# brade31919/radar_depth

Hardware: AMD Instinct MI355X
Metric: training samples/sec, resnet18_latefusion b=16 450x800 rgbd, 1/2/4/8 MI355X (higher is better)
Workload: dtype f32

## Files before the change

radar_depth_amd/csrc/norm_act.hip:

```cpp
#include "conv_internal.h"

namespace rd {

__global__ __launch_bounds__(256) void bn_finalize_kernel(const float* __restrict__ part, int n_tiles, int ld, int c0, double count,
                                                          const float* __restrict__ gamma, const float* __restrict__ beta,
                                                          float eps, float momentum, float* running_mean, float* running_var,
                                                          int64_t* nbt, float* mean, float* invstd, float* scale, float* shift) {
    const int c = blockIdx.x;
    double s = 0.0, q = 0.0;
    int t = threadIdx.x;
    for (; t + 3 * 256 < n_tiles; t += 4 * 256) {
        float a[4], b[4];
#pragma unroll
        for (int k = 0; k < 4; ++k) {
            a[k] = part[((size_t)(t + k * 256) * 2 + 0) * ld + c0 + c];
            b[k] = part[((size_t)(t + k * 256) * 2 + 1) * ld + c0 + c];
        }
#pragma unroll
        for (int k = 0; k < 4; ++k) { s += (double)a[k]; q += (double)b[k]; }
    }
    for (; t < n_tiles; t += 256) {
        s += (double)part[((size_t)t * 2 + 0) * ld + c0 + c];
        q += (double)part[((size_t)t * 2 + 1) * ld + c0 + c];
    }
// ... 49 lines not shown
}

static inline int rows_per_block(int64_t M) {
    int64_t r = cdiv64(M, 2048);
    return (int)(r < 64 ? 64 : r);
}
static inline int bwd_rows_per_block(int64_t M, int C) {
    const int RL = 256 / (C / 4) > 0 ? 256 / (C / 4) : 1;
    int64_t r = cdiv64(M, 2048);
    const int64_t lo = 4 * RL < 64 ? 4 * RL : 64;
    return (int)(r < lo ? lo : r);
}

template <int NS>
__device__ __forceinline__ void block_reduce_store(float4 (&acc)[NS], int Q, int RL, int q, int rl, bool active, float* out,
                                                   int C, float* sm) {
    if (active) {
#pragma unroll
        for (int s = 0; s < NS; ++s) *reinterpret_cast<float4*>(sm + ((size_t)(rl * NS + s) * Q + q) * 4) = acc[s];
    }
    rd_sync();
    for (int e = threadIdx.x; e < NS * Q * 4; e += blockDim.x) {
        const int s = e / (Q * 4), c = e - s * (Q * 4);
        float v = 0.f;
        for (int r = 0; r < RL; ++r) v += sm[(size_t)(r * NS + s) * Q * 4 + c];
        out[(size_t)s * C + c] = v;
    }
}

template <typename T>
__global__ __launch_bounds__(256) void bn_stats_kernel(const T* __restrict__ x, int64_t M, int C, int ldx, int RPB,
                                                       float* __restrict__ part) {
    extern __shared__ float sm[];
    const int Q = C >> 2, RL = 256 / Q;
    const int q = threadIdx.x % Q, rl = threadIdx.x / Q;
    const bool active = rl < RL;
    const int64_t r0 = (int64_t)blockIdx.x * RPB, r1 = r0 + RPB < M ? r0 + RPB : M;
    float4 acc[2] = {make_float4(0, 0, 0, 0), make_float4(0, 0, 0, 0)};
    if (active)
        for (int64_t r = r0 + rl; r < r1; r += RL) {
            const float4 v = ld4(x + r * ldx + q * 4);
            acc[0].x += v.x; acc[0].y += v.y; acc[0].z += v.z; acc[0].w += v.w;
            acc[1].x += v.x * v.x; acc[1].y += v.y * v.y; acc[1].z += v.z * v.z; acc[1].w += v.w * v.w;
        }
    block_reduce_store<2>(acc, Q, RL, q, rl, active, part + (size_t)blockIdx.x * 2 * C, C, sm);
}

template <typename T>
__global__ __launch_bounds__(256) void bn_act_kernel(const T* __restrict__ x1, int ldx1, const float* __restrict__ s1,
                                                     const float* __restrict__ t1, const T* __restrict__ x2, int ldx2,
                                                     const float* __restrict__ s2, const float* __restrict__ t2,
                                                     T* __restrict__ y, int ldy, int64_t M, int C, int act,
                                                     unsigned short* __restrict__ pc, int64_t pplane) {
    const int Q = C >> 2;
    const int lq = quad_log2(Q);
    const int64_t total = M * Q;
    for (int64_t e = (int64_t)blockIdx.x * blockDim.x + threadIdx.x; e < total; e += (int64_t)gridDim.x * blockDim.x) {
        int64_t r;
        int c;
        split_quad(e, Q, lq, r, c);
        const float4 v = ld4(x1 + r * ldx1 + c);
        const float4 a = *reinterpret_cast<const float4*>(s1 + c);
        const float4 b = *reinterpret_cast<const float4*>(t1 + c);
        float4 z = make_float4(fmaf(a.x, v.x, b.x), fmaf(a.y, v.y, b.y), fmaf(a.z, v.z, b.z), fmaf(a.w, v.w, b.w));
        if (x2) {
            float4 u = ld4(x2 + r * ldx2 + c);
            if (s2) {
                const float4 a2 = *reinterpret_cast<const float4*>(s2 + c);
                const float4 b2 = *reinterpret_cast<const float4*>(t2 + c);
                u = make_float4(fmaf(a2.x, u.x, b2.x), fmaf(a2.y, u.y, b2.y), fmaf(a2.z, u.z, b2.z), fmaf(a2.w, u.w, b2.w));
            }
            z.x += u.x; z.y += u.y; z.z += u.z; z.w += u.w;
        }
        z.x = act_fwd(z.x, act); z.y = act_fwd(z.y, act); z.z = act_fwd(z.z, act); z.w = act_fwd(z.w, act);
        st4(y + r * ldy + c, z);
        if (pc) store_pieces4(pc, pplane, M, r, c, z);
    }
}

template <typename T>
__global__ __launch_bounds__(256) void bn_bwd_reduce_kernel(const T* __restrict__ dy, int lddy, const T* __restrict__ y,
                                                            int ldy, const T* __restrict__ x1, int ldx1,
                                                            const float* __restrict__ m1, const T* __restrict__ x2, int ldx2,
                                                            const float* __restrict__ m2, T* __restrict__ g, int ldg,
                                                            int64_t M, int C, int act, int RPB, float* __restrict__ part,
                                                            const float* __restrict__ s1, const float* __restrict__ t1,
                                                            const float* __restrict__ s2, const float* __restrict__ t2) {
    extern __shared__ float sm[];
    const int Q = C >> 2, RL = 256 / Q;
    const int q = threadIdx.x % Q, rl = threadIdx.x / Q;
    const bool active = rl < RL;
    const int64_t r0 = (int64_t)blockIdx.x * RPB, r1 = r0 + RPB < M ? r0 + RPB : M;
    float4 acc[3] = {make_float4(0, 0, 0, 0), make_float4(0, 0, 0, 0), make_float4(0, 0, 0, 0)};
    if (active) {
        const int c = q * 4;
        const float4 mu1 = x1 ? *reinterpret_cast<const float4*>(m1 + c) : make_float4(0, 0, 0, 0);
        const float4 mu2 = x2 ? *reinterpret_cast<const float4*>(m2 + c) : make_float4(0, 0, 0, 0);
        const bool from_x = act != RD_ACT_NONE && !y;
        const float4 sa = from_x ? *reinterpret_cast<const float4*>(s1 + c) : make_float4(0, 0, 0, 0);
        const float4 sb = from_x ? *reinterpret_cast<const float4*>(t1 + c) : make_float4(0, 0, 0, 0);
        const bool from_x2 = from_x && x2 && s2;
        const float4 sa2 = from_x2 ? *reinterpret_cast<const float4*>(s2 + c) : make_float4(0, 0, 0, 0);
        const float4 sb2 = from_x2 ? *reinterpret_cast<const float4*>(t2 + c) : make_float4(0, 0, 0, 0);
        for (int64_t r = r0 + rl; r < r1; r += RL) {
            float4 gv = ld4(dy + r * lddy + c);
            float4 v = make_float4(0, 0, 0, 0), v2 = make_float4(0, 0, 0, 0);
            if (x1) v = ld4(x1 + r * ldx1 + c);
            if (x2) v2 = ld4(x2 + r * ldx2 + c);
            if (act != RD_ACT_NONE) {
                float4 yv;
                if (from_x) {
                    yv = make_float4(fmaf(sa.x, v.x, sb.x), fmaf(sa.y, v.y, sb.y), fmaf(sa.z, v.z, sb.z), fmaf(sa.w, v.w, sb.w));
                    if (from_x2) {
                        yv.x += fmaf(sa2.x, v2.x, sb2.x); yv.y += fmaf(sa2.y, v2.y, sb2.y);
                        yv.z += fmaf(sa2.z, v2.z, sb2.z); yv.w += fmaf(sa2.w, v2.w, sb2.w);
                    }
                } else yv = ld4(y + r * ldy + c);
                gv.x *= act_grad_from_out(yv.x, act); gv.y *= act_grad_from_out(yv.y, act);
                gv.z *= act_grad_from_out(yv.z, act); gv.w *= act_grad_from_out(yv.w, act);
            }
            if (g) st4(g + r * ldg + c, gv);
            acc[0].x += gv.x; acc[0].y += gv.y; acc[0].z += gv.z; acc[0].w += gv.w;
            if (x1) {
                acc[1].x += gv.x * (v.x - mu1.x); acc[1].y += gv.y * (v.y - mu1.y);
                acc[1].z += gv.z * (v.z - mu1.z); acc[1].w += gv.w * (v.w - mu1.w);
            }
            if (x2) {
                acc[2].x += gv.x * (v2.x - mu2.x); acc[2].y += gv.y * (v2.y - mu2.y);
                acc[2].z += gv.z * (v2.z - mu2.z); acc[2].w += gv.w * (v2.w - mu2.w);
            }
        }
    }
    block_reduce_store<3>(acc, Q, RL, q, rl, active, part + (size_t)blockIdx.x * 3 * C, C, sm);
}

__global__ __launch_bounds__(256) void bn_bwd_coeffs_kernel(const float* __restrict__ part, int n_tiles, int C, int which,
                                                            double count, const float* __restrict__ gamma,
                                                            const float* __restrict__ invstd, float* dgamma, float* dbeta,
                                                            float* coef) {
    const int c = blockIdx.x;
    double s0 = 0.0, s1 = 0.0;
    int t = threadIdx.x;
    for (; t + 3 * 256 < n_tiles; t += 4 * 256) {
        float a[4], b[4];
#pragma unroll
        for (int k = 0; k < 4; ++k) {
            a[k] = part[((size_t)(t + k * 256) * 3 + 0) * C + c];
            b[k] = part[((size_t)(t + k * 256) * 3 + which) * C + c];
        }
#pragma unroll
        for (int k = 0; k < 4; ++k) { s0 += (double)a[k]; s1 += (double)b[k]; }
    }
    for (; t < n_tiles; t += 256) {
        s0 += (double)part[((size_t)t * 3 + 0) * C + c];
        s1 += (double)part[((size_t)t * 3 + which) * C + c];
    }
    __shared__ double sh[2][4];
    s0 = wave_sum_d(s0);
    s1 = wave_sum_d(s1);
    const int w = threadIdx.x >> 6;
    if ((threadIdx.x & 63) == 0) { sh[0][w] = s0; sh[1][w] = s1; }
    rd_sync();
    if (threadIdx.x == 0) {
// ... 231 lines not shown
                    st4(g + ix, d4);
                } else if (g) {
                    st4(g + ix, o4);
                }
                if (part) {
                    acc[0].x += o4.x; acc[0].y += o4.y; acc[0].z += o4.z; acc[0].w += o4.w;
                    acc[1].x += o4.x * (vv.x - mu.x); acc[1].y += o4.y * (vv.y - mu.y);
                    acc[1].z += o4.z * (vv.z - mu.z); acc[1].w += o4.w * (vv.w - mu.w);
                }
            }
    }
    if (part) block_reduce_store<3>(acc, Q, 256 / Q, threadIdx.x % Q, threadIdx.x / Q, true, part + (size_t)blockIdx.x * 3 * C, C, sm);
}

static int ew_grid(int64_t elems) {
    int64_t g = cdiv64(elems, 256);
    const int64_t cap = (int64_t)num_cus() * 16;
    if (g > cap) g = cap;
    return (int)(g < 1 ? 1 : g);
}

static inline bool quads_ok(int C) { return C >= 4 && C % 4 == 0; }
static inline bool ld_ok(const void* p, int ld, int C) { return !p || (ld % 4 == 0 && ld >= C); }

}
using namespace rd;

extern "C" int rd_bn_finalize(const float* stat_partial, int32_t n_tiles, int32_t ld, int32_t c0, int32_t C, int64_t count, const float* gamma,
                              const float* beta, float eps, float momentum, float* running_mean, float* running_var,
                              int64_t* nbt, float* mean, float* invstd, float* scale, float* shift, void* stream) {
    RD_CHECK_ARG(n_tiles > 0 && quads_ok(C) && count > 0, "bn_finalize: bad shape (n_tiles %d, C %d)", n_tiles, C);
    RD_CHECK_ARG(c0 >= 0 && ld % 4 == 0 && (int64_t)c0 + C <= ld, "bn_finalize: channels [%d, %d + %d) outside ld = %d", c0, c0, C, ld);
    RD_CHECK_ARG(stat_partial && gamma && beta && mean && invstd && scale && shift && (!running_mean == !running_var),
                 "bn_finalize: null pointer");
    hipLaunchKernelGGL(bn_finalize_kernel, dim3(C), dim3(256), 0, static_cast<hipStream_t>(stream), stat_partial, n_tiles, ld, c0,
                       (double)count, gamma, beta, eps, momentum, running_mean, running_var, nbt, mean, invstd, scale, shift);
    RD_CHECK_LAUNCH("bn_finalize_kernel");
    return RD_OK;
}

extern "C" int rd_bn_eval_coeffs(int32_t C, const float* gamma, const float* beta, const float* running_mean,
                                 const float* running_var, float eps, float* scale, float* shift, void* stream) {
    RD_CHECK_ARG(C > 0 && gamma && beta && running_mean && running_var && scale && shift, "bn_eval_coeffs: bad arguments");
    hipLaunchKernelGGL(bn_eval_coeffs_kernel, dim3(cdiv(C, 256)), dim3(256), 0, static_cast<hipStream_t>(stream), C, gamma, beta,
                       running_mean, running_var, eps, scale, shift);
    RD_CHECK_LAUNCH("bn_eval_coeffs_kernel");
// ... 54 lines not shown
}
extern "C" int rd_bn_act_t(int32_t dtype, const void* x1, int32_t ldx1, const float* scale1, const float* shift1, const void* x2, int32_t ldx2, const float* scale2, const float* shift2, void* y, int32_t ldy, int64_t M, int32_t C, int32_t act, void* stream) {
    if (dtype == RD_DTYPE_F32) return rd_bn_act_T<float>(static_cast<const float*>(x1), ldx1, scale1, shift1, static_cast<const float*>(x2), ldx2, scale2, shift2, static_cast<float*>(y), ldy, M, C, act, stream);
    if (dtype == RD_DTYPE_BF16) return rd_bn_act_T<bf16s>(static_cast<const bf16s*>(x1), ldx1, scale1, shift1, static_cast<const bf16s*>(x2), ldx2, scale2, shift2, static_cast<bf16s*>(y), ldy, M, C, act, stream);
    rd::set_error("rd_bn_act_t: bad dtype %d", dtype);
    return RD_EINVAL;
}

template <typename T>
static int bn_bwd_reduce_impl(const T* dy, int32_t lddy, const T* y, int32_t ldy, const T* x1, int32_t ldx1,
                              const float* mean1, const T* x2, int32_t ldx2, const float* mean2, T* g, int32_t ldg,
                              int64_t M, int32_t C, int32_t act, float* red_partial, const float* scale1, const float* shift1,
                              void* stream, const float* scale2 = nullptr, const float* shift2 = nullptr, bool two_bn = false) {
    RD_CHECK_ARG(M > 0 && quads_ok(C) && C <= 1024, "bn_bwd_reduce: bad shape (C %d)", C);
    RD_CHECK_ARG(lddy % 4 == 0 && lddy >= C && ld_ok(y, ldy, C) && ld_ok(x1, ldx1, C) && ld_ok(x2, ldx2, C) && ld_ok(g, ldg, C),
                 "bn_bwd_reduce: bad stride");
    RD_CHECK_ARG(dy && red_partial, "bn_bwd_reduce: null pointer");
    RD_CHECK_ARG(!two_bn || (x1 && x2 && scale1 && shift1 && scale2 && shift2 && act != RD_ACT_NONE), "bn_bwd_reduce_x2: bad arguments");
    RD_CHECK_ARG(act == RD_ACT_NONE || y || (scale1 && shift1 && x1 && (!x2 || (scale2 && shift2))),
                 "bn_bwd_reduce: activation needs y (or the scale/shift of every operand)");
    RD_CHECK_ARG((!x1 || mean1) && (!x2 || mean2), "bn_bwd_reduce: x without mean");
    const int RPB = bwd_rows_per_block(M, C), grid = (int)cdiv64(M, RPB);
    const int Q = C / 4, RL = 256 / Q;
    hipLaunchKernelGGL(bn_bwd_reduce_kernel, dim3(grid), dim3(256), (size_t)RL * 3 * C * sizeof(float),
                       static_cast<hipStream_t>(stream), dy, lddy, y, ldy, x1, ldx1, mean1, x2, ldx2, mean2, g, ldg, M, C, act, RPB,
                       red_partial, scale1, shift1, scale2, shift2);
    RD_CHECK_LAUNCH("bn_bwd_reduce_kernel");
    return RD_OK;
}
template <typename T>
static int rd_bn_bwd_reduce_T(const T* dy, int32_t lddy, const T* y, int32_t ldy, const T* x1, int32_t ldx1, const float* mean1, const T* x2, int32_t ldx2, const float* mean2, T* g, int32_t ldg, int64_t M, int32_t C, int32_t act, float* red_partial, void* stream) {
    return bn_bwd_reduce_impl<T>(dy, lddy, y, ldy, x1, ldx1, mean1, x2, ldx2, mean2, g, ldg, M, C, act, red_partial, nullptr, nullptr, stream);
}
extern "C" int rd_bn_bwd_reduce(const float* dy, int32_t lddy, const float* y, int32_t ldy, const float* x1, int32_t ldx1, const float* mean1, const float* x2, int32_t ldx2, const float* mean2, float* g, int32_t ldg, int64_t M, int32_t C, int32_t act, float* red_partial, void* stream) {
    return rd_bn_bwd_reduce_T<float>(dy, lddy, y, ldy, x1, ldx1, mean1, x2, ldx2, mean2, g, ldg, M, C, act, red_partial, stream);
}
extern "C" int rd_bn_bwd_reduce_t(int32_t dtype, const void* dy, int32_t lddy, const void* y, int32_t ldy, const void* x1, int32_t ldx1, const float* mean1, const void* x2, int32_t ldx2, const float* mean2, void* g, int32_t ldg, int64_t M, int32_t C, int32_t act, float* red_partial, void* stream) {
    if (dtype == RD_DTYPE_F32) return rd_bn_bwd_reduce_T<float>(static_cast<const float*>(dy), lddy, static_cast<const float*>(y), ldy, static_cast<const float*>(x1), ldx1, mean1, static_cast<const float*>(x2), ldx2, mean2, static_cast<float*>(g), ldg, M, C, act, red_partial, stream);
    if (dtype == RD_DTYPE_BF16) return rd_bn_bwd_reduce_T<bf16s>(static_cast<const bf16s*>(dy), lddy, static_cast<const bf16s*>(y), ldy, static_cast<const bf16s*>(x1), ldx1, mean1, static_cast<const bf16s*>(x2), ldx2, mean2, static_cast<bf16s*>(g), ldg, M, C, act, red_partial, stream);
    rd::set_error("rd_bn_bwd_reduce_t: bad dtype %d", dtype);
    return RD_EINVAL;
}
template <typename T>
static int rd_bn_bwd_reduce_x_T(const T* dy, int32_t lddy, const T* x1, int32_t ldx1, const float* mean1, const float* scale1, const float* shift1, T* g, int32_t ldg, int64_t M, int32_t C, int32_t act, float* red_partial, void* stream) {
    return bn_bwd_reduce_impl<T>(dy, lddy, nullptr, 0, x1, ldx1, mean1, nullptr, 0, nullptr, g, ldg, M, C, act, red_partial, scale1, shift1, stream);
}
extern "C" int rd_bn_bwd_reduce_x(const float* dy, int32_t lddy, const float* x1, int32_t ldx1, const float* mean1, const float* scale1, const float* shift1, float* g, int32_t ldg, int64_t M, int32_t C, int32_t act, float* red_partial, void* stream) {
    return rd_bn_bwd_reduce_x_T<float>(dy, lddy, x1, ldx1, mean1, scale1, shift1, g, ldg, M, C, act, red_partial, stream);
}
extern "C" int rd_bn_bwd_reduce_x_t(int32_t dtype, const void* dy, int32_t lddy, const void* x1, int32_t ldx1, const float* mean1, const float* scale1, const float* shift1, void* g, int32_t ldg, int64_t M, int32_t C, int32_t act, float* red_partial, void* stream) {
    if (dtype == RD_DTYPE_F32) return rd_bn_bwd_reduce_x_T<float>(static_cast<const float*>(dy), lddy, static_cast<const float*>(x1), ldx1, mean1, scale1, shift1, static_cast<float*>(g), ldg, M, C, act, red_partial, stream);
    if (dtype == RD_DTYPE_BF16) return rd_bn_bwd_reduce_x_T<bf16s>(static_cast<const bf16s*>(dy), lddy, static_cast<const bf16s*>(x1), ldx1, mean1, scale1, shift1, static_cast<bf16s*>(g), ldg, M, C, act, red_partial, stream);
    rd::set_error("rd_bn_bwd_reduce_x_t: bad dtype %d", dtype);
    return RD_EINVAL;
}

namespace rd {
int launch_bn_bwd_coeffs(const float* red_partial, int n_tiles, int C, int which, double count, const float* gamma, const float* invstd,
                         float* dgamma, float* dbeta, float* coef_ws, hipStream_t s) {
    hipLaunchKernelGGL(bn_bwd_coeffs_kernel, dim3(C), dim3(256), 0, s, red_partial, n_tiles, C, which, count, gamma, invstd, dgamma, dbeta,
                       coef_ws);
    RD_CHECK_LAUNCH("bn_bwd_coeffs_kernel");
    return RD_OK;
}
}

template <typename T>
static int rd_bn_bwd_apply_T(const T* g, int32_t ldg, const T* x, int32_t ldx, const float* red_partial, int32_t n_tiles, int32_t which, const float* gamma, const float* mean, const float* invstd, float* dgamma, float* dbeta, float* coef_ws, T* dx, int32_t lddx, int64_t M, int32_t C, void* stream,
                             void* pieces = nullptr, int64_t piece_elems = 0) {
    RD_CHECK_ARG((which == 1 || which == 2) && M > 0 && n_tiles > 0 && quads_ok(C), "bn_bwd_apply: bad shape (which %d, n_tiles %d, C %d)",
                 which, n_tiles, C);
    RD_CHECK_ARG(ldg % 4 == 0 && ldg >= C && ldx % 4 == 0 && ldx >= C && lddx % 4 == 0 && lddx >= C, "bn_bwd_apply: bad stride");
    RD_CHECK_ARG(g && x && red_partial && gamma && mean && invstd && coef_ws && dx, "bn_bwd_apply: null pointer");
    RD_CHECK_ARG(!pieces || piece_planes_ok(pieces, piece_elems, M, C), "bn_bwd_apply: bad piece planes");
    hipStream_t s = static_cast<hipStream_t>(stream);
    hipLaunchKernelGGL(bn_bwd_coeffs_kernel, dim3(C), dim3(256), 0, s, red_partial, n_tiles, C, which, (double)M, gamma, invstd,
                       dgamma, dbeta, coef_ws);
    RD_CHECK_LAUNCH("bn_bwd_coeffs_kernel");
    hipLaunchKernelGGL((bn_bwd_dx_kernel<T>), dim3(ew_grid(M * (C / 4))), dim3(256), 0, s, g, ldg, x, ldx, mean, coef_ws, dx, lddx, M, C,
                       (const float*)nullptr, (const float*)nullptr, RD_ACT_NONE, static_cast<unsigned short*>(pieces), piece_elems);
    RD_CHECK_LAUNCH("bn_bwd_dx_kernel");
    return RD_OK;
}
extern "C" int rd_bn_bwd_apply(const float* g, int32_t ldg, const float* x, int32_t ldx, const float* red_partial, int32_t n_tiles, int32_t which, const float* gamma, const float* mean, const float* invstd, float* dgamma, float* dbeta, float* coef_ws, float* dx, int32_t lddx, int64_t M, int32_t C, void* stream) {
    return rd_bn_bwd_apply_T<float>(g, ldg, x, ldx, red_partial, n_tiles, which, gamma, mean, invstd, dgamma, dbeta, coef_ws, dx, lddx, M, C, stream);
}
extern "C" int rd_bn_bwd_apply_p(const float* g, int32_t ldg, const float* x, int32_t ldx, const float* red_partial, int32_t n_tiles, int32_t which, const float* gamma, const float* mean, const float* invstd, float* dgamma, float* dbeta, float* coef_ws, float* dx, int32_t lddx, int64_t M, int32_t C, void* pieces, int64_t piece_elems, void* stream) {
    return rd_bn_bwd_apply_T<float>(g, ldg, x, ldx, red_partial, n_tiles, which, gamma, mean, invstd, dgamma, dbeta, coef_ws, dx, lddx, M, C, stream, pieces, piece_elems);
}
extern "C" int rd_bn_bwd_apply_t(int32_t dtype, const void* g, int32_t ldg, const void* x, int32_t ldx, const float* red_partial, int32_t n_tiles, int32_t which, const float* gamma, const float* mean, const float* invstd, float* dgamma, float* dbeta, float* coef_ws, void* dx, int32_t lddx, int64_t M, int32_t C, void* stream) {
    if (dtype == RD_DTYPE_F32) return rd_bn_bwd_apply_T<float>(static_cast<const float*>(g), ldg, static_cast<const float*>(x), ldx, red_partial, n_tiles, which, gamma, mean, invstd, dgamma, dbeta, coef_ws, static_cast<float*>(dx), lddx, M, C, stream);
    if (dtype == RD_DTYPE_BF16) return rd_bn_bwd_apply_T<bf16s>(static_cast<const bf16s*>(g), ldg, static_cast<const bf16s*>(x), ldx, red_partial, n_tiles, which, gamma, mean, invstd, dgamma, dbeta, coef_ws, static_cast<bf16s*>(dx), lddx, M, C, stream);
    rd::set_error("rd_bn_bwd_apply_t: bad dtype %d", dtype);
    return RD_EINVAL;
}

template <typename T>
static int rd_bn_bwd_reduce_x2_T(const T* dy, int32_t lddy, const T* x1, int32_t ldx1, const float* mean1, const float* scale1, const float* shift1, const T* x2, int32_t ldx2, const float* mean2, const float* scale2, const float* shift2, int64_t M, int32_t C, int32_t act, float* red_partial, void* stream) {
    return bn_bwd_reduce_impl<T>(dy, lddy, nullptr, 0, x1, ldx1, mean1, x2, ldx2, mean2, nullptr, 0, M, C, act, red_partial, scale1, shift1, stream,
                              scale2, shift2, true);
}
extern "C" int rd_bn_bwd_reduce_x2(const float* dy, int32_t lddy, const float* x1, int32_t ldx1, const float* mean1, const float* scale1, const float* shift1, const float* x2, int32_t ldx2, const float* mean2, const float* scale2, const float* shift2, int64_t M, int32_t C, int32_t act, float* red_partial, void* stream) {
    return rd_bn_bwd_reduce_x2_T<float>(dy, lddy, x1, ldx1, mean1, scale1, shift1, x2, ldx2, mean2, scale2, shift2, M, C, act, red_partial, stream);
}
extern "C" int rd_bn_bwd_reduce_x2_t(int32_t dtype, const void* dy, int32_t lddy, const void* x1, int32_t ldx1, const float* mean1, const float* scale1, const float* shift1, const void* x2, int32_t ldx2, const float* mean2, const float* scale2, const float* shift2, int64_t M, int32_t C, int32_t act, float* red_partial, void* stream) {
    if (dtype == RD_DTYPE_F32) return rd_bn_bwd_reduce_x2_T<float>(static_cast<const float*>(dy), lddy, static_cast<const float*>(x1), ldx1, mean1, scale1, shift1, static_cast<const float*>(x2), ldx2, mean2, scale2, shift2, M, C, act, red_partial, stream);
    if (dtype == RD_DTYPE_BF16) return rd_bn_bwd_reduce_x2_T<bf16s>(static_cast<const bf16s*>(dy), lddy, static_cast<const bf16s*>(x1), ldx1, mean1, scale1, shift1, static_cast<const bf16s*>(x2), ldx2, mean2, scale2, shift2, M, C, act, red_partial, stream);
    rd::set_error("rd_bn_bwd_reduce_x2_t: bad dtype %d", dtype);
    return RD_EINVAL;
}
template <typename T>
static int rd_bn_bwd_apply_x2_T(const T* dy, int32_t lddy, const T* x1, int32_t ldx1, const T* x2, int32_t ldx2, const float* red_partial, int32_t n_tiles, const float* gamma1, const float* mean1, const float* invstd1, const float* scale1, const float* shift1, const float* gamma2, const float* mean2, const float* invstd2, const float* scale2, const float* shift2, int32_t act, float* dgamma1, float* dbeta1, float* dgamma2, float* dbeta2, float* coef_ws6, T* dx1, int32_t lddx1, T* dx2, int32_t lddx2, int64_t M, int32_t C, void* stream,
                                void* pieces1 = nullptr, int64_t piece_elems1 = 0, void* pieces2 = nullptr, int64_t piece_elems2 = 0) {
    RD_CHECK_ARG(M > 0 && n_tiles > 0 && quads_ok(C), "bn_bwd_apply_x2: bad shape (n_tiles %d, C %d)", n_tiles, C);
    RD_CHECK_ARG(lddy % 4 == 0 && lddy >= C && ldx1 % 4 == 0 && ldx1 >= C && ldx2 % 4 == 0 && ldx2 >= C && lddx1 % 4 == 0 && lddx1 >= C &&
                     lddx2 % 4 == 0 && lddx2 >= C, "bn_bwd_apply_x2: bad stride");
    RD_CHECK_ARG(dy && x1 && x2 && red_partial && gamma1 && gamma2 && mean1 && mean2 && invstd1 && invstd2 && scale1 && shift1 && scale2 &&
                     shift2 && coef_ws6 && dx1 && dx2, "bn_bwd_apply_x2: null pointer");
    RD_CHECK_ARG((!pieces1 || piece_planes_ok(pieces1, piece_elems1, M, C)) && (!pieces2 || piece_planes_ok(pieces2, piece_elems2, M, C)), "bn_bwd_apply_x2: bad piece planes");
    hipStream_t s = static_cast<hipStream_t>(stream);
    hipLaunchKernelGGL(bn_bwd_coeffs_kernel, dim3(C), dim3(256), 0, s, red_partial, n_tiles, C, 1, (double)M, gamma1, invstd1, dgamma1, dbeta1,
                       coef_ws6);
    RD_CHECK_LAUNCH("bn_bwd_coeffs_kernel");
    hipLaunchKernelGGL(bn_bwd_coeffs_kernel, dim3(C), dim3(256), 0, s, red_partial, n_tiles, C, 2, (double)M, gamma2, invstd2, dgamma2, dbeta2,
                       coef_ws6 + 3 * C);
    RD_CHECK_LAUNCH("bn_bwd_coeffs_kernel");
    hipLaunchKernelGGL((bn_bwd_dx2_kernel<T>), dim3(ew_grid(M * (C / 4))), dim3(256), 0, s, dy, lddy, x1, ldx1, x2, ldx2, mean1, mean2, coef_ws6,
                       coef_ws6 + 3 * C, scale1, shift1, scale2, shift2, act, dx1, lddx1, dx2, lddx2, M, C,
                       static_cast<unsigned short*>(pieces1), piece_elems1, static_cast<unsigned short*>(pieces2), piece_elems2);
    RD_CHECK_LAUNCH("bn_bwd_dx2_kernel");
    return RD_OK;
}
extern "C" int rd_bn_bwd_apply_x2(const float* dy, int32_t lddy, const float* x1, int32_t ldx1, const float* x2, int32_t ldx2, const float* red_partial, int32_t n_tiles, const float* gamma1, const float* mean1, const float* invstd1, const float* scale1, const float* shift1, const float* gamma2, const float* mean2, const float* invstd2, const float* scale2, const float* shift2, int32_t act, float* dgamma1, float* dbeta1, float* dgamma2, float* dbeta2, float* coef_ws6, float* dx1, int32_t lddx1, float* dx2, int32_t lddx2, int64_t M, int32_t C, void* stream) {
    return rd_bn_bwd_apply_x2_T<float>(dy, lddy, x1, ldx1, x2, ldx2, red_partial, n_tiles, gamma1, mean1, invstd1, scale1, shift1, gamma2, mean2, invstd2, scale2, shift2, act, dgamma1, dbeta1, dgamma2, dbeta2, coef_ws6, dx1, lddx1, dx2, lddx2, M, C, stream);
}
extern "C" int rd_bn_bwd_apply_x2_p(const float* dy, int32_t lddy, const float* x1, int32_t ldx1, const float* x2, int32_t ldx2, const float* red_partial, int32_t n_tiles, const float* gamma1, const float* mean1, const float* invstd1, const float* scale1, const float* shift1, const float* gamma2, const float* mean2, const float* invstd2, const float* scale2, const float* shift2, int32_t act, float* dgamma1, float* dbeta1, float* dgamma2, float* dbeta2, float* coef_ws6, float* dx1, int32_t lddx1, float* dx2, int32_t lddx2, int64_t M, int32_t C, void* pieces1, int64_t piece_elems1, void* pieces2, int64_t piece_elems2, void* stream) {
    return rd_bn_bwd_apply_x2_T<float>(dy, lddy, x1, ldx1, x2, ldx2, red_partial, n_tiles, gamma1, mean1, invstd1, scale1, shift1, gamma2, mean2, invstd2, scale2, shift2, act, dgamma1, dbeta1, dgamma2, dbeta2, coef_ws6, dx1, lddx1, dx2, lddx2, M, C, stream, pieces1, piece_elems1, pieces2, piece_elems2);
}
extern "C" int rd_bn_bwd_apply_x2_t(int32_t dtype, const void* dy, int32_t lddy, const void* x1, int32_t ldx1, const void* x2, int32_t ldx2, const float* red_partial, int32_t n_tiles, const float* gamma1, const float* mean1, const float* invstd1, const float* scale1, const float* shift1, const float* gamma2, const float* mean2, const float* invstd2, const float* scale2, const float* shift2, int32_t act, float* dgamma1, float* dbeta1, float* dgamma2, float* dbeta2, float* coef_ws6, void* dx1, int32_t lddx1, void* dx2, int32_t lddx2, int64_t M, int32_t C, void* stream) {
    if (dtype == RD_DTYPE_F32) return rd_bn_bwd_apply_x2_T<float>(static_cast<const float*>(dy), lddy, static_cast<const float*>(x1), ldx1, static_cast<const float*>(x2), ldx2, red_partial, n_tiles, gamma1, mean1, invstd1, scale1, shift1, gamma2, mean2, invstd2, scale2, shift2, act, dgamma1, dbeta1, dgamma2, dbeta2, coef_ws6, static_cast<float*>(dx1), lddx1, static_cast<float*>(dx2), lddx2, M, C, stream);
    if (dtype == RD_DTYPE_BF16) return rd_bn_bwd_apply_x2_T<bf16s>(static_cast<const bf16s*>(dy), lddy, static_cast<const bf16s*>(x1), ldx1, static_cast<const bf16s*>(x2), ldx2, red_partial, n_tiles, gamma1, mean1, invstd1, scale1, shift1, gamma2, mean2, invstd2, scale2, shift2, act, dgamma1, dbeta1, dgamma2, dbeta2, coef_ws6, static_cast<bf16s*>(dx1), lddx1, static_cast<bf16s*>(dx2), lddx2, M, C, stream);
    rd::set_error("rd_bn_bwd_apply_x2_t: bad dtype %d", dtype);
    return RD_EINVAL;
}

template <typename T>
static int rd_bn_bwd_apply_x_T(const T* dy, int32_t lddy, const T* x, int32_t ldx, const float* red_partial, int32_t n_tiles, const float* gamma, const float* mean, const float* invstd, const float* scale, const float* shift, int32_t act, float* dgamma, float* dbeta, float* coef_ws, T* dx, int32_t lddx, int64_t M, int32_t C, void* stream,
                               void* pieces = nullptr, int64_t piece_elems = 0) {
    RD_CHECK_ARG(M > 0 && n_tiles > 0 && quads_ok(C), "bn_bwd_apply_x: bad shape (n_tiles %d, C %d)", n_tiles, C);
    RD_CHECK_ARG(lddy % 4 == 0 && lddy >= C && ldx % 4 == 0 && ldx >= C && lddx % 4 == 0 && lddx >= C, "bn_bwd_apply_x: bad stride");
    RD_CHECK_ARG(dy && x && red_partial && gamma && mean && invstd && scale && shift && coef_ws && dx, "bn_bwd_apply_x: null pointer");
    RD_CHECK_ARG(!pieces || piece_planes_ok(pieces, piece_elems, M, C), "bn_bwd_apply_x: bad piece planes");
    hipStream_t s = static_cast<hipStream_t>(stream);
    hipLaunchKernelGGL(bn_bwd_coeffs_kernel, dim3(C), dim3(256), 0, s, red_partial, n_tiles, C, 1, (double)M, gamma, invstd, dgamma,
                       dbeta, coef_ws);
    RD_CHECK_LAUNCH("bn_bwd_coeffs_kernel");
    hipLaunchKernelGGL((bn_bwd_dx_kernel<T>), dim3(ew_grid(M * (C / 4))), dim3(256), 0, s, dy, lddy, x, ldx, mean, coef_ws, dx, lddx, M, C,
                       scale, shift, act, static_cast<unsigned short*>(pieces), piece_elems);
    RD_CHECK_LAUNCH("bn_bwd_dx_kernel");
    return RD_OK;
}
extern "C" int rd_bn_bwd_apply_x(const float* dy, int32_t lddy, const float* x, int32_t ldx, const float* red_partial, int32_t n_tiles, const float* gamma, const float* mean, const float* invstd, const float* scale, const float* shift, int32_t act, float* dgamma, float* dbeta, float* coef_ws, float* dx, int32_t lddx, int64_t M, int32_t C, void* stream) {
    return rd_bn_bwd_apply_x_T<float>(dy, lddy, x, ldx, red_partial, n_tiles, gamma, mean, invstd, scale, shift, act, dgamma, dbeta, coef_ws, dx, lddx, M, C, stream);
}
extern "C" int rd_bn_bwd_apply_x_p(const float* dy, int32_t lddy, const float* x, int32_t ldx, const float* red_partial, int32_t n_tiles, const float* gamma, const float* mean, const float* invstd, const float* scale, const float* shift, int32_t act, float* dgamma, float* dbeta, float* coef_ws, float* dx, int32_t lddx, int64_t M, int32_t C, void* pieces, int64_t piece_elems, void* stream) {
    return rd_bn_bwd_apply_x_T<float>(dy, lddy, x, ldx, red_partial, n_tiles, gamma, mean, invstd, scale, shift, act, dgamma, dbeta, coef_ws, dx, lddx, M, C, stream, pieces, piece_elems);
}
extern "C" int rd_bn_bwd_apply_x_t(int32_t dtype, const void* dy, int32_t lddy, const void* x, int32_t ldx, const float* red_partial, int32_t n_tiles, const float* gamma, const float* mean, const float* invstd, const float* scale, const float* shift, int32_t act, float* dgamma, float* dbeta, float* coef_ws, void* dx, int32_t lddx, int64_t M, int32_t C, void* stream) {
    if (dtype == RD_DTYPE_F32) return rd_bn_bwd_apply_x_T<float>(static_cast<const float*>(dy), lddy, static_cast<const float*>(x), ldx, red_partial, n_tiles, gamma, mean, invstd, scale, shift, act, dgamma, dbeta, coef_ws, static_cast<float*>(dx), lddx, M, C, stream);
    if (dtype == RD_DTYPE_BF16) return rd_bn_bwd_apply_x_T<bf16s>(static_cast<const bf16s*>(dy), lddy, static_cast<const bf16s*>(x), ldx, red_partial, n_tiles, gamma, mean, invstd, scale, shift, act, dgamma, dbeta, coef_ws, static_cast<bf16s*>(dx), lddx, M, C, stream);
    rd::set_error("rd_bn_bwd_apply_x_t: bad dtype %d", dtype);
    return RD_EINVAL;
}

template <typename T>
static int rd_bnact_maxpool_fwd_T(const T* x, const float* scale, const float* shift, int32_t act, int32_t N, int32_t H, int32_t W, int32_t C, T* y, int32_t ldy, uint8_t* idx, void* stream,
                                  void* pieces = nullptr, int64_t piece_elems = 0) {
    RD_CHECK_ARG(N > 0 && H > 0 && W > 0 && quads_ok(C), "bnact_maxpool_fwd: bad shape (%d, %d, %d, C %d)", N, H, W, C);
    RD_CHECK_ARG(ldy % 4 == 0 && ldy >= C, "bnact_maxpool_fwd: bad stride %d", ldy);
// ... 62 lines not shown
extern "C" int rd_bnact_maxpool_bwd_stats(const float* dy, int32_t lddy, const uint8_t* idx, const float* x, const float* scale, const float* shift, int32_t act, int32_t N, int32_t H, int32_t W, int32_t C, float* g, const float* mean, float* red_partial, void* stream) {
    return rd_bnact_maxpool_bwd_stats_T<float>(dy, lddy, idx, x, scale, shift, act, N, H, W, C, g, mean, red_partial, stream);
}
extern "C" int rd_bnact_maxpool_bwd_stats_t(int32_t dtype, const void* dy, int32_t lddy, const uint8_t* idx, const void* x, const float* scale, const float* shift, int32_t act, int32_t N, int32_t H, int32_t W, int32_t C, void* g, const float* mean, float* red_partial, void* stream) {
    if (dtype == RD_DTYPE_F32) return rd_bnact_maxpool_bwd_stats_T<float>(static_cast<const float*>(dy), lddy, idx, static_cast<const float*>(x), scale, shift, act, N, H, W, C, static_cast<float*>(g), mean, red_partial, stream);
    if (dtype == RD_DTYPE_BF16) return rd_bnact_maxpool_bwd_stats_T<bf16s>(static_cast<const bf16s*>(dy), lddy, idx, static_cast<const bf16s*>(x), scale, shift, act, N, H, W, C, static_cast<bf16s*>(g), mean, red_partial, stream);
    rd::set_error("rd_bnact_maxpool_bwd_stats_t: bad dtype %d", dtype);
    return RD_EINVAL;
}

template <typename T>
static int rd_bnact_maxpool_bwd_apply_T(const T* dy, int32_t lddy, const uint8_t* idx, const T* x, const float* scale, const float* shift,
                                        int32_t act, int32_t N, int32_t H, int32_t W, int32_t C, const float* red_partial, int32_t n_tiles,
                                        const float* gamma, const float* mean, const float* invstd, float* dgamma, float* dbeta,
                                        float* coef_ws, T* dx, void* stream) {
    RD_CHECK_ARG(N > 0 && H > 0 && W > 0 && n_tiles > 0 && quads_ok(C), "bnact_maxpool_bwd_apply: bad shape (%d, %d, %d, n_tiles %d, C %d)", N, H,
                 W, n_tiles, C);
    RD_CHECK_ARG(256 % (C / 4) == 0, "bnact_maxpool_bwd_apply: C/4 = %d must divide 256", C / 4);
    RD_CHECK_ARG(lddy % 4 == 0 && lddy >= C, "bnact_maxpool_bwd_apply: bad stride %d", lddy);
    RD_CHECK_ARG(dy && idx && x && scale && shift && red_partial && gamma && mean && invstd && coef_ws && dx,
                 "bnact_maxpool_bwd_apply: null pointer");
    const int Ho = (H + 2 - 3) / 2 + 1, Wo = (W + 2 - 3) / 2 + 1;
    hipStream_t s = static_cast<hipStream_t>(stream);
    hipLaunchKernelGGL(bn_bwd_coeffs_kernel, dim3(C), dim3(256), 0, s, red_partial, n_tiles, C, 1, (double)((int64_t)N * H * W), gamma, invstd,
                       dgamma, dbeta, coef_ws);
    RD_CHECK_LAUNCH("bn_bwd_coeffs_kernel");
    hipLaunchKernelGGL((bnact_maxpool_bwd_kernel<T>), dim3(ew_grid((int64_t)N * Ho * Wo * (C / 4))), dim3(256), 0, s, dy, lddy, idx, x, scale,
                       shift, act, N, H, W, C, Ho, Wo, dx, mean, (float*)nullptr, (const float*)coef_ws);
    RD_CHECK_LAUNCH("bnact_maxpool_bwd_kernel");
    return RD_OK;
}
extern "C" int rd_bnact_maxpool_bwd_apply_t(int32_t dtype, const void* dy, int32_t lddy, const uint8_t* idx, const void* x, const float* scale,
                                            const float* shift, int32_t act, int32_t N, int32_t H, int32_t W, int32_t C,
                                            const float* red_partial, int32_t n_tiles, const float* gamma, const float* mean,
                                            const float* invstd, float* dgamma, float* dbeta, float* coef_ws, void* dx, void* stream) {
    if (dtype == RD_DTYPE_F32)
        return rd_bnact_maxpool_bwd_apply_T<float>(static_cast<const float*>(dy), lddy, idx, static_cast<const float*>(x), scale, shift, act, N, H, W, C,
                                                   red_partial, n_tiles, gamma, mean, invstd, dgamma, dbeta, coef_ws, static_cast<float*>(dx), stream);
    if (dtype == RD_DTYPE_BF16)
        return rd_bnact_maxpool_bwd_apply_T<bf16s>(static_cast<const bf16s*>(dy), lddy, idx, static_cast<const bf16s*>(x), scale, shift, act, N, H, W, C,
                                                   red_partial, n_tiles, gamma, mean, invstd, dgamma, dbeta, coef_ws, static_cast<bf16s*>(dx), stream);
    rd::set_error("rd_bnact_maxpool_bwd_apply_t: bad dtype %d", dtype);
    return RD_EINVAL;
}
```

Measured before the change: 1087.

## Specialize BN backward reduce by source mode and unroll row loops

Templates the BN backward reduction kernel on activation source (none, from y, recomputed from x1 or x1+x2) and on x1/x2 presence, picks the instantiation on the host, and unrolls row loads with a register-budget-derived factor plus occupancy-tuned launch bounds. It also unrolls the BN stats row loop and the shared-memory column reduction, and merges the two per-input coefficient launches in the dual-input apply path into one 2-D grid. The aim is to remove per-row runtime branches, expose more memory-level parallelism and cut one launch. In exchange it adds many kernel instantiations and more register pressure, and assumes the activation gradient is a sign-dependent constant (ReLU/leaky).

After: 1088 (median of 6 runs). About the same (+0.1%).

```diff
diff --git a/radar_depth_amd/csrc/norm_act.hip b/radar_depth_amd/csrc/norm_act.hip
--- a/radar_depth_amd/csrc/norm_act.hip
+++ b/radar_depth_amd/csrc/norm_act.hip
@@ -95,10 +95,36 @@
     rd_sync();
     for (int e = threadIdx.x; e < NS * Q * 4; e += blockDim.x) {
         const int s = e / (Q * 4), c = e - s * (Q * 4);
+        const float* col = sm + (size_t)s * Q * 4 + c;
+        const int step = NS * Q * 4;
         float v = 0.f;
-        for (int r = 0; r < RL; ++r) v += sm[(size_t)(r * NS + s) * Q * 4 + c];
+        int r = 0;
+#pragma unroll 1
+        for (; r + 8 <= RL; r += 8) {
+            float t[8];
+#pragma unroll
+            for (int k = 0; k < 8; ++k) t[k] = col[(size_t)(r + k) * step];
+#pragma unroll
+            for (int k = 0; k < 8; ++k) v += t[k];
+        }
+        for (; r < RL; ++r) v += col[(size_t)r * step];
         out[(size_t)s * C + c] = v;
     }
+}
+
+template <typename T, int U>
+__device__ __forceinline__ int64_t bn_stats_trips(const T* __restrict__ x, int ldx, int64_t r, int64_t r1, int RL, float4 (&acc)[2]) {
+    for (; r + (int64_t)(U - 1) * RL < r1; r += (int64_t)U * RL) {
+        float4 v[U];
+#pragma unroll
+        for (int k = 0; k < U; ++k) v[k] = ld4(x + (r + (int64_t)k * RL) * ldx);
+#pragma unroll
+        for (int k = 0; k < U; ++k) {
+            acc[0].x += v[k].x; acc[0].y += v[k].y; acc[0].z += v[k].z; acc[0].w += v[k].w;
+            acc[1].x += v[k].x * v[k].x; acc[1].y += v[k].y * v[k].y; acc[1].z += v[k].z * v[k].z; acc[1].w += v[k].w * v[k].w;
+        }
+    }
+    return r;
 }
 
 template <typename T>
@@ -110,12 +136,10 @@
     const bool active = rl < RL;
     const int64_t r0 = (int64_t)blockIdx.x * RPB, r1 = r0 + RPB < M ? r0 + RPB : M;
     float4 acc[2] = {make_float4(0, 0, 0, 0), make_float4(0, 0, 0, 0)};
-    if (active)
-        for (int64_t r = r0 + rl; r < r1; r += RL) {
-            const float4 v = ld4(x + r * ldx + q * 4);
-            acc[0].x += v.x; acc[0].y += v.y; acc[0].z += v.z; acc[0].w += v.w;
-            acc[1].x += v.x * v.x; acc[1].y += v.y * v.y; acc[1].z += v.z * v.z; acc[1].w += v.w * v.w;
-        }
+    if (active) {
+        const int64_t r = bn_stats_trips<T, 4>(x + q * 4, ldx, r0 + rl, r1, RL, acc);
+        bn_stats_trips<T, 1>(x + q * 4, ldx, r, r1, RL, acc);
+    }
     block_reduce_store<2>(acc, Q, RL, q, rl, active, part + (size_t)blockIdx.x * 2 * C, C, sm);
 }
 
@@ -151,14 +175,101 @@
     }
 }
 
-template <typename T>
-__global__ __launch_bounds__(256) void bn_bwd_reduce_kernel(const T* __restrict__ dy, int lddy, const T* __restrict__ y,
-                                                            int ldy, const T* __restrict__ x1, int ldx1,
-                                                            const float* __restrict__ m1, const T* __restrict__ x2, int ldx2,
-                                                            const float* __restrict__ m2, T* __restrict__ g, int ldg,
-                                                            int64_t M, int C, int act, int RPB, float* __restrict__ part,
-                                                            const float* __restrict__ s1, const float* __restrict__ t1,
-                                                            const float* __restrict__ s2, const float* __restrict__ t2) {
+enum BwdSrc { BWD_NOACT = 0, BWD_FROM_Y = 1, BWD_FROM_X1 = 2, BWD_FROM_X12 = 3 };
+
+template <typename T>
+struct BwdRows {
+    const T *dy, *y, *x1, *x2;
+    T* g;
+    int64_t sdy, sy, sx1, sx2, sg;
+    bool has_g;
+    float neg;
+};
+struct BwdCoef { float4 mu1, mu2, sa, sb, sa2, sb2; };
+
+template <typename T, int SRC, bool X1, bool X2>
+__device__ __forceinline__ void bn_bwd_reduce_row(const BwdCoef& k, float neg, T* g, float4 gv, const float4 v, const float4 v2, float4 yv,
+                                                  float4 (&acc)[3]) {
+    if (SRC != BWD_NOACT) {
+        if (SRC >= BWD_FROM_X1) {
+            yv = make_float4(fmaf(k.sa.x, v.x, k.sb.x), fmaf(k.sa.y, v.y, k.sb.y), fmaf(k.sa.z, v.z, k.sb.z), fmaf(k.sa.w, v.w, k.sb.w));
+            if (SRC == BWD_FROM_X12) {
+                yv.x += fmaf(k.sa2.x, v2.x, k.sb2.x); yv.y += fmaf(k.sa2.y, v2.y, k.sb2.y);
+                yv.z += fmaf(k.sa2.z, v2.z, k.sb2.z); yv.w += fmaf(k.sa2.w, v2.w, k.sb2.w);
+            }
+        }
+        gv.x *= yv.x > 0.f ? 1.f : neg; gv.y *= yv.y > 0.f ? 1.f : neg;
+        gv.z *= yv.z > 0.f ? 1.f : neg; gv.w *= yv.w > 0.f ? 1.f : neg;
+    }
+    if (g) st4(g, gv);
+    acc[0].x += gv.x; acc[0].y += gv.y; acc[0].z += gv.z; acc[0].w += gv.w;
+    if (X1) {
+        acc[1].x += gv.x * (v.x - k.mu1.x); acc[1].y += gv.y * (v.y - k.mu1.y);
+        acc[1].z += gv.z * (v.z - k.mu1.z); acc[1].w += gv.w * (v.w - k.mu1.w);
+    }
+    if (X2) {
+        acc[2].x += gv.x * (v2.x - k.mu2.x); acc[2].y += gv.y * (v2.y - k.mu2.y);
+        acc[2].z += gv.z * (v2.z - k.mu2.z); acc[2].w += gv.w * (v2.w - k.mu2.w);
+    }
+}
+
+template <typename T, int U, int SRC, bool X1, bool X2>
+__device__ __forceinline__ int bn_bwd_reduce_trips(BwdRows<T>& a, const BwdCoef& co, int i, int n, int RL, float4 (&acc)[3]) {
+    const float4 zero = make_float4(0, 0, 0, 0);
+#pragma unroll 1
+    for (; i + (U - 1) * RL < n; i += U * RL) {
+        float4 gv[U], v[U], v2[U], yv[U];
+#pragma unroll
+        for (int k = 0; k < U; ++k) {
+            gv[k] = ld4(a.dy + k * a.sdy);
+            v[k] = X1 ? ld4(a.x1 + k * a.sx1) : zero;
+            v2[k] = X2 ? ld4(a.x2 + k * a.sx2) : zero;
+            yv[k] = SRC == BWD_FROM_Y ? ld4(a.y + k * a.sy) : zero;
+        }
+#pragma unroll
+        for (int k = 0; k < U; ++k)
+            bn_bwd_reduce_row<T, SRC, X1, X2>(co, a.neg, a.has_g ? a.g + k * a.sg : nullptr, gv[k], v[k], v2[k], yv[k], acc);
+        a.dy += U * a.sdy;
+        if (X1) a.x1 += U * a.sx1;
+        if (X2) a.x2 += U * a.sx2;
+        if (SRC == BWD_FROM_Y) a.y += U * a.sy;
+        if (a.has_g) a.g += U * a.sg;
+    }
+    return i;
+}
+
+template <typename T, int SRC, bool X1, bool X2>
+__device__ __forceinline__ void bn_bwd_reduce_rows(const BwdRows<T>& k, int64_t r, int c, const float* m1, const float* m2, const float* s1,
+                                                   const float* t1, const float* s2, const float* t2, int rl, int n, int RL,
+                                                   float4 (&acc)[3]) {
+    const float4 zero = make_float4(0, 0, 0, 0);
+    BwdCoef co;
+    co.mu1 = X1 ? *reinterpret_cast<const float4*>(m1) : zero;
+    co.mu2 = X2 ? *reinterpret_cast<const float4*>(m2) : zero;
+    co.sa = SRC >= BWD_FROM_X1 ? *reinterpret_cast<const float4*>(s1) : zero;
+    co.sb = SRC >= BWD_FROM_X1 ? *reinterpret_cast<const float4*>(t1) : zero;
+    co.sa2 = SRC == BWD_FROM_X12 ? *reinterpret_cast<const float4*>(s2) : zero;
+    co.sb2 = SRC == BWD_FROM_X12 ? *reinterpret_cast<const float4*>(t2) : zero;
+    constexpr int NX = (X1 ? 1 : 0) + (X2 ? 1 : 0);
+    constexpr int ROW = 4 * (1 + (SRC == BWD_FROM_Y ? 1 : 0) + NX);
+    constexpr int KEPT = 4 * (1 + NX) + 4 * (NX + (SRC >= BWD_FROM_X1 ? 2 : 0));
+    constexpr int U = SRC == BWD_FROM_X12 ? 2 : KEPT + 4 * ROW <= 20 ? 4 : KEPT + 3 * ROW <= 36 ? 3 : KEPT + 2 * ROW <= 36 ? 2 : 1;
+    BwdRows<T> a = k;
+    a.dy += r * k.sdy + c; a.sdy *= RL;
+    if (SRC == BWD_FROM_Y) { a.y += r * k.sy + c; a.sy *= RL; }
+    if (X1) { a.x1 += r * k.sx1 + c; a.sx1 *= RL; }
+    if (X2) { a.x2 += r * k.sx2 + c; a.sx2 *= RL; }
+    if (k.has_g) { a.g += r * k.sg + c; a.sg *= RL; }
+    const int i = bn_bwd_reduce_trips<T, U, SRC, X1, X2>(a, co, rl, n, RL, acc);
+    bn_bwd_reduce_trips<T, 1, SRC, X1, X2>(a, co, i, n, RL, acc);
+}
+
+template <typename T, int SRC, bool X1, bool X2>
+__global__ __launch_bounds__(256, SRC == BWD_FROM_X12 ? 1 : 8) void bn_bwd_reduce_kernel(
+    const T* __restrict__ dy, int lddy, const T* __restrict__ y, int ldy, const T* __restrict__ x1, int ldx1, const float* __restrict__ m1,
+    const T* __restrict__ x2, int ldx2, const float* __restrict__ m2, T* __restrict__ g, int ldg, int64_t M, int C, int act, int RPB,
+    float* __restrict__ part, const float* __restrict__ s1, const float* __restrict__ t1, const float* __restrict__ s2,
+    const float* __restrict__ t2) {
     extern __shared__ float sm[];
     const int Q = C >> 2, RL = 256 / Q;
     const int q = threadIdx.x % Q, rl = threadIdx.x / Q;
@@ -167,51 +278,38 @@
     float4 acc[3] = {make_float4(0, 0, 0, 0), make_float4(0, 0, 0, 0), make_float4(0, 0, 0, 0)};
     if (active) {
         const int c = q * 4;
-        const float4 mu1 = x1 ? *reinterpret_cast<const float4*>(m1 + c) : make_float4(0, 0, 0, 0);
-        const float4 mu2 = x2 ? *reinterpret_cast<const float4*>(m2 + c) : make_float4(0, 0, 0, 0);
-        const bool from_x = act != RD_ACT_NONE && !y;
-        const float4 sa = from_x ? *reinterpret_cast<const float4*>(s1 + c) : make_float4(0, 0, 0, 0);
-        const float4 sb = from_x ? *reinterpret_cast<const float4*>(t1 + c) : make_float4(0, 0, 0, 0);
-        const bool from_x2 = from_x && x2 && s2;
-        const float4 sa2 = from_x2 ? *reinterpret_cast<const float4*>(s2 + c) : make_float4(0, 0, 0, 0);
-        const float4 sb2 = from_x2 ? *reinterpret_cast<const float4*>(t2 + c) : make_float4(0, 0, 0, 0);
-        for (int64_t r = r0 + rl; r < r1; r += RL) {
-            float4 gv = ld4(dy + r * lddy + c);
-            float4 v = make_float4(0, 0, 0, 0), v2 = make_float4(0, 0, 0, 0);
-            if (x1) v = ld4(x1 + r * ldx1 + c);
-            if (x2) v2 = ld4(x2 + r * ldx2 + c);
-            if (act != RD_ACT_NONE) {
-                float4 yv;
-                if (from_x) {
-                    yv = make_float4(fmaf(sa.x, v.x, sb.x), fmaf(sa.y, v.y, sb.y), fmaf(sa.z, v.z, sb.z), fmaf(sa.w, v.w, sb.w));
-                    if (from_x2) {
-                        yv.x += fmaf(sa2.x, v2.x, sb2.x); yv.y += fmaf(sa2.y, v2.y, sb2.y);
-                        yv.z += fmaf(sa2.z, v2.z, sb2.z); yv.w += fmaf(sa2.w, v2.w, sb2.w);
-                    }
-                } else yv = ld4(y + r * ldy + c);
-                gv.x *= act_grad_from_out(yv.x, act); gv.y *= act_grad_from_out(yv.y, act);
-                gv.z *= act_grad_from_out(yv.z, act); gv.w *= act_grad_from_out(yv.w, act);
-            }
-            if (g) st4(g + r * ldg + c, gv);
-            acc[0].x += gv.x; acc[0].y += gv.y; acc[0].z += gv.z; acc[0].w += gv.w;
-            if (x1) {
-                acc[1].x += gv.x * (v.x - mu1.x); acc[1].y += gv.y * (v.y - mu1.y);
-                acc[1].z += gv.z * (v.z - mu1.z); acc[1].w += gv.w * (v.w - mu1.w);
-            }
-            if (x2) {
-                acc[2].x += gv.x * (v2.x - mu2.x); acc[2].y += gv.y * (v2.y - mu2.y);
-                acc[2].z += gv.z * (v2.z - mu2.z); acc[2].w += gv.w * (v2.w - mu2.w);
-            }
-        }
+        BwdRows<T> a;
+        a.dy = dy; a.y = y; a.x1 = x1; a.x2 = x2; a.g = g;
+        a.sdy = lddy; a.sy = ldy; a.sx1 = ldx1; a.sx2 = ldx2; a.sg = ldg;
+        a.has_g = g != nullptr;
+        a.neg = act_grad_from_out(-1.f, act);
+        bn_bwd_reduce_rows<T, SRC, X1, X2>(a, r0 + rl, c, m1 + c, m2 + c, s1 + c, t1 + c, s2 + c, t2 + c, rl, (int)(r1 - r0), RL, acc);
     }
     block_reduce_store<3>(acc, Q, RL, q, rl, active, part + (size_t)blockIdx.x * 3 * C, C, sm);
 }
 
-__global__ __launch_bounds__(256) void bn_bwd_coeffs_kernel(const float* __restrict__ part, int n_tiles, int C, int which,
-                                                            double count, const float* __restrict__ gamma,
-                                                            const float* __restrict__ invstd, float* dgamma, float* dbeta,
-                                                            float* coef) {
-    const int c = blockIdx.x;
+template <typename T>
+static decltype(&bn_bwd_reduce_kernel<T, BWD_NOACT, false, false>) bn_bwd_reduce_form(int act, bool y, bool x1, bool x2, bool s2) {
+#define RD_BWD_FORMS(SRC) (x1 ? (x2 ? bn_bwd_reduce_kernel<T, SRC, true, true> : bn_bwd_reduce_kernel<T, SRC, true, false>) \
+                              : (x2 ? bn_bwd_reduce_kernel<T, SRC, false, true> : bn_bwd_reduce_kernel<T, SRC, false, false>))
+    if (act == RD_ACT_NONE) return RD_BWD_FORMS(BWD_NOACT);
+    if (y) return RD_BWD_FORMS(BWD_FROM_Y);
+#undef RD_BWD_FORMS
+    if (x2 && s2) return bn_bwd_reduce_kernel<T, BWD_FROM_X12, true, true>;
+    return x2 ? bn_bwd_reduce_kernel<T, BWD_FROM_X1, true, true> : bn_bwd_reduce_kernel<T, BWD_FROM_X1, true, false>;
+}
+
+struct BwdCoefJob {
+    int which;
+    const float *gamma, *invstd;
+    float *dgamma, *dbeta, *coef;
+};
+__global__ __launch_bounds__(256) void bn_bwd_coeffs_kernel(const float* __restrict__ part, int n_tiles, int C, double count, BwdCoefJob j0,
+                                                            BwdCoefJob j1) {
+    const BwdCoefJob j = blockIdx.y ? j1 : j0;
+    const int c = blockIdx.x, which = j.which;
+    const float *gamma = j.gamma, *invstd = j.invstd;
+    float *dgamma = j.dgamma, *dbeta = j.dbeta, *coef = j.coef;
     double s0 = 0.0, s1 = 0.0;
     int t = threadIdx.x;
     for (; t + 3 * 256 < n_tiles; t += 4 * 256) {
@@ -489,6 +587,12 @@
 
 static inline bool quads_ok(int C) { return C >= 4 && C % 4 == 0; }
 static inline bool ld_ok(const void* p, int ld, int C) { return !p || (ld % 4 == 0 && ld >= C); }
+static int launch_bwd_coeffs(const float* red_partial, int n_tiles, int C, double count, const BwdCoefJob& j0, const BwdCoefJob* j1,
+                             hipStream_t s) {
+    hipLaunchKernelGGL(bn_bwd_coeffs_kernel, dim3(C, j1 ? 2 : 1), dim3(256), 0, s, red_partial, n_tiles, C, count, j0, j1 ? *j1 : j0);
+    RD_CHECK_LAUNCH("bn_bwd_coeffs_kernel");
+    return RD_OK;
+}
 
 }
 using namespace rd;
@@ -589,9 +693,9 @@
     RD_CHECK_ARG((!x1 || mean1) && (!x2 || mean2), "bn_bwd_reduce: x without mean");
     const int RPB = bwd_rows_per_block(M, C), grid = (int)cdiv64(M, RPB);
     const int Q = C / 4, RL = 256 / Q;
-    hipLaunchKernelGGL(bn_bwd_reduce_kernel, dim3(grid), dim3(256), (size_t)RL * 3 * C * sizeof(float),
-                       static_cast<hipStream_t>(stream), dy, lddy, y, ldy, x1, ldx1, mean1, x2, ldx2, mean2, g, ldg, M, C, act, RPB,
-                       red_partial, scale1, shift1, scale2, shift2);
+    const auto kernel = bn_bwd_reduce_form<T>(act, y != nullptr, x1 != nullptr, x2 != nullptr, scale2 != nullptr);
+    hipLaunchKernelGGL(kernel, dim3(grid), dim3(256), (size_t)RL * 3 * C * sizeof(float), static_cast<hipStream_t>(stream), dy, lddy, y,
+                       ldy, x1, ldx1, mean1, x2, ldx2, mean2, g, ldg, M, C, act, RPB, red_partial, scale1, shift1, scale2, shift2);
     RD_CHECK_LAUNCH("bn_bwd_reduce_kernel");
     return RD_OK;
 }
@@ -625,10 +729,7 @@
 namespace rd {
 int launch_bn_bwd_coeffs(const float* red_partial, int n_tiles, int C, int which, double count, const float* gamma, const float* invstd,
                          float* dgamma, float* dbeta, float* coef_ws, hipStream_t s) {
-    hipLaunchKernelGGL(bn_bwd_coeffs_kernel, dim3(C), dim3(256), 0, s, red_partial, n_tiles, C, which, count, gamma, invstd, dgamma, dbeta,
-                       coef_ws);
-    RD_CHECK_LAUNCH("bn_bwd_coeffs_kernel");
-    return RD_OK;
+    return launch_bwd_coeffs(red_partial, n_tiles, C, count, BwdCoefJob{which, gamma, invstd, dgamma, dbeta, coef_ws}, nullptr, s);
 }
 }
 
@@ -641,9 +742,7 @@
     RD_CHECK_ARG(g && x && red_partial && gamma && mean && invstd && coef_ws && dx, "bn_bwd_apply: null pointer");
     RD_CHECK_ARG(!pieces || piece_planes_ok(pieces, piece_elems, M, C), "bn_bwd_apply: bad piece planes");
     hipStream_t s = static_cast<hipStream_t>(stream);
-    hipLaunchKernelGGL(bn_bwd_coeffs_kernel, dim3(C), dim3(256), 0, s, red_partial, n_tiles, C, which, (double)M, gamma, invstd,
-                       dgamma, dbeta, coef_ws);
-    RD_CHECK_LAUNCH("bn_bwd_coeffs_kernel");
+    if (int rc = launch_bwd_coeffs(red_partial, n_tiles, C, (double)M, BwdCoefJob{which, gamma, invstd, dgamma, dbeta, coef_ws}, nullptr, s)) return rc;
     hipLaunchKernelGGL((bn_bwd_dx_kernel<T>), dim3(ew_grid(M * (C / 4))), dim3(256), 0, s, g, ldg, x, ldx, mean, coef_ws, dx, lddx, M, C,
                        (const float*)nullptr, (const float*)nullptr, RD_ACT_NONE, static_cast<unsigned short*>(pieces), piece_elems);
     RD_CHECK_LAUNCH("bn_bwd_dx_kernel");
@@ -686,12 +785,8 @@
                      shift2 && coef_ws6 && dx1 && dx2, "bn_bwd_apply_x2: null pointer");
     RD_CHECK_ARG((!pieces1 || piece_planes_ok(pieces1, piece_elems1, M, C)) && (!pieces2 || piece_planes_ok(pieces2, piece_elems2, M, C)), "bn_bwd_apply_x2: bad piece planes");
     hipStream_t s = static_cast<hipStream_t>(stream);
-    hipLaunchKernelGGL(bn_bwd_coeffs_kernel, dim3(C), dim3(256), 0, s, red_partial, n_tiles, C, 1, (double)M, gamma1, invstd1, dgamma1, dbeta1,
-                       coef_ws6);
-    RD_CHECK_LAUNCH("bn_bwd_coeffs_kernel");
-    hipLaunchKernelGGL(bn_bwd_coeffs_kernel, dim3(C), dim3(256), 0, s, red_partial, n_tiles, C, 2, (double)M, gamma2, invstd2, dgamma2, dbeta2,
-                       coef_ws6 + 3 * C);
-    RD_CHECK_LAUNCH("bn_bwd_coeffs_kernel");
+    const BwdCoefJob j1{1, gamma1, invstd1, dgamma1, dbeta1, coef_ws6}, j2{2, gamma2, invstd2, dgamma2, dbeta2, coef_ws6 + 3 * C};
+    if (int rc = launch_bwd_coeffs(red_partial, n_tiles, C, (double)M, j1, &j2, s)) return rc;
     hipLaunchKernelGGL((bn_bwd_dx2_kernel<T>), dim3(ew_grid(M * (C / 4))), dim3(256), 0, s, dy, lddy, x1, ldx1, x2, ldx2, mean1, mean2, coef_ws6,
                        coef_ws6 + 3 * C, scale1, shift1, scale2, shift2, act, dx1, lddx1, dx2, lddx2, M, C,
                        static_cast<unsigned short*>(pieces1), piece_elems1, static_cast<unsigned short*>(pieces2), piece_elems2);
@@ -719,9 +814,7 @@
     RD_CHECK_ARG(dy && x && red_partial && gamma && mean && invstd && scale && shift && coef_ws && dx, "bn_bwd_apply_x: null pointer");
     RD_CHECK_ARG(!pieces || piece_planes_ok(pieces, piece_elems, M, C), "bn_bwd_apply_x: bad piece planes");
     hipStream_t s = static_cast<hipStream_t>(stream);
-    hipLaunchKernelGGL(bn_bwd_coeffs_kernel, dim3(C), dim3(256), 0, s, red_partial, n_tiles, C, 1, (double)M, gamma, invstd, dgamma,
-                       dbeta, coef_ws);
-    RD_CHECK_LAUNCH("bn_bwd_coeffs_kernel");
+    if (int rc = launch_bwd_coeffs(red_partial, n_tiles, C, (double)M, BwdCoefJob{1, gamma, invstd, dgamma, dbeta, coef_ws}, nullptr, s)) return rc;
     hipLaunchKernelGGL((bn_bwd_dx_kernel<T>), dim3(ew_grid(M * (C / 4))), dim3(256), 0, s, dy, lddy, x, ldx, mean, coef_ws, dx, lddx, M, C,
                        scale, shift, act, static_cast<unsigned short*>(pieces), piece_elems);
     RD_CHECK_LAUNCH("bn_bwd_dx_kernel");
@@ -830,9 +923,9 @@
                  "bnact_maxpool_bwd_apply: null pointer");
     const int Ho = (H + 2 - 3) / 2 + 1, Wo = (W + 2 - 3) / 2 + 1;
     hipStream_t s = static_cast<hipStream_t>(stream);
-    hipLaunchKernelGGL(bn_bwd_coeffs_kernel, dim3(C), dim3(256), 0, s, red_partial, n_tiles, C, 1, (double)((int64_t)N * H * W), gamma, invstd,
-                       dgamma, dbeta, coef_ws);
-    RD_CHECK_LAUNCH("bn_bwd_coeffs_kernel");
+    if (int rc = launch_bwd_coeffs(red_partial, n_tiles, C, (double)((int64_t)N * H * W), BwdCoefJob{1, gamma, invstd, dgamma, dbeta, coef_ws},
+                                   nullptr, s))
+        return rc;
     hipLaunchKernelGGL((bnact_maxpool_bwd_kernel<T>), dim3(ew_grid((int64_t)N * Ho * Wo * (C / 4))), dim3(256), 0, s, dy, lddy, idx, x, scale,
                        shift, act, N, H, W, C, Ho, Wo, dx, mean, (float*)nullptr, (const float*)coef_ws);
     RD_CHECK_LAUNCH("bnact_maxpool_bwd_kernel");
```
